# UVA-Computer-Vision-Lab/LabelAny3D

Measured on AMD Instinct MI355X. Metric: fitted 3D boxes/sec @640x480, higher is better.
Workload: dtype f64

## Files before the change

### labelany3d_amd/csrc/la3d_instance.hip

```cpp
#include <algorithm>
#include <atomic>
#include <chrono>
#include <cstdint>
#include <cstddef>
#include <cstring>
#include <mutex>
#include <type_traits>
#include <utility>
#include <vector>

#include "la3d_device.hpp"
#include "la3d_poly.hpp"
#include "la3d_engines.hpp"
#include "la3d_walks.hpp"
#include "la3d_stages.hpp"
#include "la3d_instance_phases.hpp"
#include "la3d_hull.hpp"

#ifndef LA3D_INSTANCE_DT
#define LA3D_INSTANCE_DT 0
#endif
#if LA3D_INSTANCE_DT == 0
using DepthT = float;
using KParams = la3d::FitParams;
#define LA3D_INSTANCE_FIT instance_fit
#elif LA3D_INSTANCE_DT == 1
using DepthT = la3d::d_f16;
using KParams = la3d::FitParams16;
#define LA3D_INSTANCE_FIT instance_fit_f16
#define fit_instances_kernel fit_instances_f16_kernel
#else
using DepthT = la3d::d_u16;
using KParams = la3d::FitParams16;
#define LA3D_INSTANCE_FIT instance_fit_u16
#define fit_instances_kernel fit_instances_u16_kernel
#endif

namespace {
__device__ inline const float* depth_planes(const FitParams& p, const FitParams&) { return p.depth; }
__device__ inline DepthCvt<float> depth_cvt(const FitParams&) { return {}; }
#if LA3D_INSTANCE_DT != 0
__device__ inline const DepthT* depth_planes(const FitParams&, const FitParams16& call) { return reinterpret_cast<const DepthT*>(call.depth16); }
__device__ inline DepthCvt<DepthT> depth_cvt(const FitParams16& call) {
  DepthCvt<DepthT> cv;
#if LA3D_INSTANCE_DT == 2
  cv.scale = call.d16_scale; cv.hole = call.d16_hole;
#endif
  return cv;
}
__device__ inline long long frame_depth_offset(const FitParams& call, int img) {
  const long long off_v = call.frames[img].depth_offset;
  return uniform_i64(off_v);
}
#endif
__device__ inline void sweep_sep_hull(const FitParams& p, const DepthT* __restrict__ dpl, const unsigned* bits, const unsigned short* list,
                                      int nactive, const double* Mg, unsigned* col, int wave, int lane, double px0, double pz0,
                                      double* acc, double* yext, int* cnt, const DepthCvt<DepthT> cv) {
  const int c = lane & 31, h4 = (lane >> 5) * 4;
  const double a00 = Mg[0], a02 = Mg[2], a11 = Mg[4], a12 = Mg[5];
  double s0 = acc[0], s1 = acc[1], s2 = acc[2], s3 = acc[3], s4 = acc[4], ylo = yext[0], yhi = yext[1];
  int n = *cnt;
  for (int e = wave; e < nactive; e += NWAVE) {
    const unsigned t = __builtin_amdgcn_readfirstlane((unsigned)list[e]);
    const int u = (int)(t & 0xffu) * 32 + c, v0 = (int)(t >> 8) * 8 + h4;
    const uint4 w = *reinterpret_cast<const uint4*>(bits + e * 8 + h4);
    const unsigned nib = ((w.x >> c) & 1u) | (((w.y >> c) & 1u) << 1) | (((w.z >> c) & 1u) << 2) | (((w.w >> c) & 1u) << 3);
    const double r0 = fma(a00, (double)u, a02);
    unsigned kmin = 0xffffffffu, kmax = 0u;
#pragma unroll
    for (int k = 0; k < 4; ++k) {
      const int v = v0 + k;
      if (((nib >> k) & 1u) && v < p.H) {
        const float df = depth_at<DepthT>(dpl, (long long)v * p.W + u, cv);
        if (finite_f32(df)) {
          const unsigned key = hull_key(__float_as_uint(df));
          kmin = min(kmin, key); kmax = max(kmax, key);
          const double d = (double)df;
          const double x = d * r0 - px0, z = d - pz0, y = d * fma(a11, (double)v, a12);
          s0 += x; s1 += z; s2 = fma(x, x, s2); s3 = fma(x, z, s3); s4 = fma(z, z, s4);
          ylo = fmin(ylo, y); yhi = fmax(yhi, y);
          n += 1;
        }
      }
    }
    if (kmin <= kmax) { atomicMin(col + u, kmin); atomicMax(col + p.W + u, kmax); }
  }
  acc[0] = s0; acc[1] = s1; acc[2] = s2; acc[3] = s3; acc[4] = s4; yext[0] = ylo; yext[1] = yhi;
  *cnt = n;
}

__device__ inline void hull_full_mask(Shared* sh, const FitParams& p, int inst, const DepthT* __restrict__ dpl, unsigned* bits, const unsigned short* list,
                                      int nactive, bool sep, const double* Mg, int nmask, int wave, int lane, const DepthCvt<DepthT> cv) {
  if (!sep) {
    if (tid_here(wave, lane) == 0) write_no_box(p, inst, LA3D_BOX_UNSUPPORTED, 0.0, NAN);
    return;
  }
  unsigned* col = bits + nactive * 8;
  double hacc[5] = {0, 0, 0, 0, 0}, yx[2] = {INFINITY, -INFINITY};
  int hcnt = 0;
  sweep_sep_hull(p, dpl, bits, list, nactive, Mg, col, wave, lane, 0.0, 0.0, hacc, yx, &hcnt, cv);
  stage_moments_to_axis(sh, p, inst, hacc, hcnt, nmask, tid_here(wave, lane), wave, lane, true);
  if (sh->redo) {
    __syncthreads();
    double piv[2];
    get_pivot(sh, piv);
#pragma unroll
    for (int i = 0; i < 5; ++i) hacc[i] = 0;
    hcnt = 0;
    sweep_sep_hull(p, dpl, bits, list, nactive, Mg, col, wave, lane, piv[0], piv[1], hacc, yx, &hcnt, cv);
    stage_moments_to_axis(sh, p, inst, hacc, hcnt, nmask, tid_here(wave, lane), wave, lane, false);
  }
  if (sh->st != LA3D_BOX_OK) return;
  const double ylo_w = wave_min(yx[0]), yhi_w = wave_max(yx[1]);
  if (lane == 0) { sh->part[wave][5] = ylo_w; sh->part[wave][6] = yhi_w; }
  __syncthreads();
  double* hh = hull_slot(p.geo, inst, hull_stride_bytes(false, p.W));
  unsigned* hcol = reinterpret_cast<unsigned*>(hh + HH_D);
  for (int i = tid_here(wave, lane); i < 2 * p.W; i += NT) hcol[i] = col[i];
  if (tid_here(wave, lane) == 0) {
    double ylo = INFINITY, yhi = -INFINITY;
    for (int w = 0; w < NWAVE; ++w) { ylo = fmin(ylo, sh->part[w][5]); yhi = fmax(yhi, sh->part[w][6]); }
    hull_handoff_header(hh, sh, ylo, yhi, Mg[0], Mg[2], 0.0);
  }
}

template <bool VEC, bool LDSMASK, bool SAMPLE, bool TILED, int SRC, bool HULL = false, bool FRAMES = false>
__global__ __launch_bounds__(NT, NT / 64) void fit_instances_kernel(const KParams p_call) {
  static_assert(!FRAMES || (VEC && LDSMASK && TILED && !HULL && (SRC == 1 || SRC == 2 || SRC == 3)), "frames calls: run lengths / polygons / bit planes, tiled form");
  FitParams p_frame;
  if constexpr (FRAMES) p_frame = p_call;
  const FitParams& p_block = p_call;
  const FitParams& p = FRAMES ? p_frame : p_block;
  extern __shared__ __attribute__((aligned(16))) unsigned char smem[];
  unsigned* bits = reinterpret_cast<unsigned*>(smem);
  Shared* sh = reinterpret_cast<Shared*>(smem + p_call.mask_lds_bytes);
  unsigned* prefix = reinterpret_cast<unsigned*>(smem + p_call.mask_lds_bytes + sizeof(Shared));
  unsigned short* list = reinterpret_cast<unsigned short*>(smem + p_call.mask_lds_bytes + sizeof(Shared));

  constexpr bool REBUILD_TID = TILED && !SAMPLE;
  const int tid_in = threadIdx.x;
  const int lane = REBUILD_TID ? (int)__builtin_amdgcn_mbcnt_hi(~0u, __builtin_amdgcn_mbcnt_lo(~0u, 0u)) : (tid_in & 63);
  const int wave = __builtin_amdgcn_readfirstlane(tid_in >> 6);
  const int tid = REBUILD_TID ? ((wave << 6) | lane) : tid_in;
#ifdef LA3D_TIMELINE
  const unsigned long long t_entry = wall_clock64();
#endif
  if (!FRAMES && !SAMPLE && p.order_self && (int)blockIdx.x < p.order_resident && !(p.order_self == 2 && blockIdx.x % 7 == 3)) {
    for (int ie = (int)blockIdx.x; ie < p.B; ie += p.order_resident) {
      if (ie != (int)blockIdx.x) __syncthreads();
      estimate_publish_wg<SRC == 3>(p, ie, sh, tid, wave, lane);
    }
  }
  const int inst = p.order_nch > 0 ? order_select<SRC == 3>(p, (int)blockIdx.x, sh, wave, lane) : xcd_remap(blockIdx.x, p.B);
  if (tid == 0) { sh->order_inst = inst; sh->sep_bad = 0; }
  if constexpr (HULL) { if (tid == 0) hull_slot(p.geo, inst, hull_stride_bytes(SAMPLE, p.W))[HH_STATE] = -1.0; }
  const int img = p.image_index ? p.image_index[inst] : inst;
  if constexpr (FRAMES) {
    if (!frame_geometry<true, SAMPLE>(p_frame, p_call, img) || (SRC == 3 && !frame_bits_offset_ok(p_call, inst))) {
      if (tid == 0) write_no_box(p, inst, LA3D_BOX_UNSUPPORTED, 0.0, NAN);
      return;
    }
  }
  const int HW = p.HW;
  const DepthT* dpl = depth_planes(p, p_call) + (long long)img * p.depth_plane_stride;
#if LA3D_INSTANCE_DT != 0
  if constexpr (FRAMES) dpl += frame_depth_offset(p_call, img);
#endif
  const DepthCvt<DepthT> cv = depth_cvt(p_call);
  const unsigned char* mpl = p.mask ? p.mask + (long long)inst * HW : nullptr;

  if (tid == NT - 1) {
    double Kinv[9], Rg[9];
    inv3_camera(p.K + (long long)img * p.k_stride, Kinv);
    sh->bad_ground = ground_rotation(p.ground ? p.ground + (long long)inst * 4 : nullptr, Rg);
#pragma unroll
    for (int i = 0; i < 3; ++i)
#pragma unroll
      for (int j = 0; j < 3; ++j) sh->M[i * 3 + j] = Rg[i] * Kinv[j] + Rg[3 + i] * Kinv[3 + j] + Rg[6 + i] * Kinv[6 + j];
#pragma unroll
    for (int i = 0; i < 9; ++i) sh->Rg[i] = Rg[i];
  }

#ifdef LA3D_TIMELINE
  double* tl = p.geo + 1024 + (long long)inst * 16;
#define LA3D_STAMP(k) do { if (tid == 0) tl[k] = (double)wall_clock64(); } while (0)
  if (tid == 0) { tl[7] = (double)blockIdx.x; tl[8] = (double)t_entry; sh->tl = tl; }
#else
#define LA3D_STAMP(k) do { } while (0)
#endif
  LA3D_STAMP(0);
  if (!SAMPLE && p.stagger_ticks > 0 && p.order_nch > 0 && blockIdx.x < 1024) {
    const unsigned long long t0 = wall_clock64();
    const unsigned g = blockIdx.x >> 8;
    const unsigned long long w = (unsigned long long)p.stagger_ticks * (g == 1 ? 13u : (g == 2 ? 29u : (g == 3 ? 47u : 0u))) / 16u;
    while (wall_clock64() - t0 < w) __builtin_amdgcn_s_sleep(32);
  }
  int my_draw = 0;
  if (SAMPLE && tid < LA3D_NSAMPLE) my_draw = p.sample_idx[(long long)inst * LA3D_NSAMPLE + tid];
  int nmask = 0;
  if constexpr (LDSMASK) nmask = mask_to_bits<VEC, SRC, FRAMES>(p, p_call, inst, mpl, bits, sh, list, TILED ? p.list_cap / 2 : 0, tid, wave, lane);
  __syncthreads();
  LA3D_STAMP(1);
  const int inst_p = __builtin_amdgcn_readfirstlane(sh->order_inst);
  if constexpr (FRAMES) frame_geometry<false, SAMPLE>(p_frame, p_call, p.image_index[inst_p]);
  const int tid_plain = tid;
#define tid (REBUILD_TID ? tid_here(wave, lane) : tid_plain)
  if (SRC != 0 && LDSMASK && p.filter_boundary >= 0) {
    if (!filter_keep<SRC>(p, sh, bits, inst_p, tid)) return;
  }
  double Mg[9];
#pragma unroll
  for (int i = 0; i < 9; ++i) Mg[i] = uniform_f64(sh->M[i]);
  LA3D_STAMP(13);

  bool sampled = false;
  int ntot = 0;
  if (SAMPLE) {
    const int wsum = wave_sum_i(nmask);
    if (lane == 0) sh->nmask[wave] = wsum;
    __syncthreads();
    for (int w = 0; w < NWAVE; ++w) ntot += sh->nmask[w];
    sampled = HULL || ntot > LA3D_NSAMPLE;
  }

  constexpr bool LK = TILED && !SAMPLE;
  const bool sep_cam = LK && (HULL || !p.sep_off) && Mg[1] == 0.0 && Mg[3] == 0.0 && Mg[6] == 0.0 && Mg[7] == 0.0 && Mg[8] == 1.0;
  TileList tiles;
  if (TILED && !sampled) {
    if constexpr (FRAMES) frame_rcp_ntx(p_frame);
    tiles = build_tile_list<LK>(p, sh, bits, list, sep_cam, tid, wave, lane);
    LA3D_STAMP(15);
    __syncthreads();
  }
  const int nactive = tiles.nactive, nfull = tiles.nfull, compact = tiles.compact;
  const bool sep = tiles.sep;

  if constexpr (HULL && LK) {
    hull_full_mask(sh, p, inst_p, dpl, bits, list, nactive, sep, Mg, nmask, wave, lane, cv);
    return;
  }

  if constexpr (LK) {
    if (sep) {
      LA3D_STAMP(2);
      unsigned* col = bits + nactive * 8;
      double sacc[5] = {0, 0, 0, 0, 0}, yx[2] = {INFINITY, -INFINITY};
      unsigned unsafe = 0u;
      if (p.H & 7) sweep_sep<true>(p, dpl, bits, list, nactive, Mg, col, wave, lane, sacc, yx, &unsafe, 0, nfull, cv);
      else sweep_sep<false>(p, dpl, bits, list, nactive, Mg, col, wave, lane, sacc, yx, &unsafe, 0, nfull, cv);
      if (__ballot(unsafe >= 0x7f800000u) != 0ull && lane == 0) sh->sep_bad = 1;
      const double ylo_w = uniform_f64(wave_min(yx[0])), yhi_w = uniform_f64(wave_max(yx[1]));
      LA3D_STAMP(3);
      stage_moments_to_axis(sh, p, inst_p, sacc, nmask, nmask, tid, wave, lane, true);
      LA3D_STAMP(4);
      if (!(sh->redo || sh->sep_bad)) {
        if (sh->st != LA3D_BOX_OK) return;
        double N0[3], N2[3], ext[6];
        yaw_rows(sh, Mg, N0, N2);
        sep_col_extents(col, p.W, N0, N2, tid, ext);
        ext[2] = ylo_w; ext[3] = yhi_w;
        LA3D_STAMP(5);
        if constexpr (FRAMES) frame_proj(p_frame, p_call, inst_p);
        stage_extents_to_box(sh, p, inst_p, ext, tid, wave, lane);
        stage_status_aux(sh, p, inst_p, tid);
        LA3D_STAMP(6);
        return;
      }
      __syncthreads();
    }
  }

  bool cull = false;
  int rng_words = 0;
  if constexpr (LK) {
    if (compact) {
      rng_words = cull_rng_words(nactive);
      cull = nactive >= p.cull_min && nactive <= CULL_MAXT;
      if (!cull) {
        unsigned short* surv = reinterpret_cast<unsigned short*>(bits + nactive * 8);
#pragma clang loop vectorize(disable) interleave(disable) unroll(disable)
        for (int t = tid; t < nactive; t += NT) surv[t] = (unsigned short)t;
      }
    }
  }

  LA3D_STAMP(2);
  double acc[5] = {0, 0, 0, 0, 0};
  int cnt = 0;
  double px = 0, py = 0, pz = 0;
  bool pok = false;

  if (SAMPLE) {
    if (sampled) {
      sample_pick<HULL, FRAMES, DepthT>(p, sh, bits, prefix, dpl, cv, Mg, ntot, my_draw, tid, wave, lane, acc, &cnt, &px, &py, &pz, &pok);
    }
  }
  bool checked = !TILED;
  if (!sampled) {
    if (TILED) {
      constexpr bool SP = !SAMPLE;
      const bool specA = SP && Mg[6] == 0.0 && Mg[7] == 0.0 && Mg[8] == 1.0;
      if (LK && cull) {
        if (specA) sweep_tiled<0, false, true, SP>(p, dpl, bits, list, nactive, Mg, Mg + 3, Mg + 6, wave, lane, acc, &cnt, nullptr, compact, rng_words, -1, nfull, cv);
        else sweep_tiled<0, false, true>(p, dpl, bits, list, nactive, Mg, Mg + 3, Mg + 6, wave, lane, acc, &cnt, nullptr, compact, rng_words, -1, nfull, cv);
      } else {
        if (specA) sweep_tiled<0, false, false, SP>(p, dpl, bits, list, nactive, Mg, Mg + 3, Mg + 6, wave, lane, acc, &cnt, nullptr, compact, rng_words, -1, nfull, cv);
        else sweep_tiled<0, false>(p, dpl, bits, list, nactive, Mg, Mg + 3, Mg + 6, wave, lane, acc, &cnt, nullptr, compact, rng_words, -1, nfull, cv);
      }
      cnt = nmask;
    }
    else sweep<VEC, LDSMASK, 0>(p, dpl, mpl, bits, Mg, Mg + 3, Mg + 6, wave, lane, acc, &cnt, &nmask, nullptr, cv);
  }

  LA3D_STAMP(3);
  stage_moments_to_axis(sh, p, inst_p, acc, cnt, nmask, tid, wave, lane, true);
  if (sh->redo) {
    __syncthreads();
#pragma unroll
    for (int i = 0; i < 5; ++i) acc[i] = 0;
    cnt = 0;
    if (sampled) {
      if (pok) {
        const double x = px - pivot_ptr(sh)[0], z = pz - pivot_ptr(sh)[1];
        acc[0] = x; acc[1] = z; acc[2] = x * x; acc[3] = x * z; acc[4] = z * z;
        cnt = 1;
      }
    } else if (TILED) {
      if (sh->redo == 2) {
        pivot_pass(p, dpl, bits, list, nactive, Mg, Mg + 6, wave, lane, compact, pivot_ptr(sh), acc, &cnt, cv);
      } else {
        checked = true;
        if (LK && cull) sweep_tiled<0, true, true>(p, dpl, bits, list, nactive, Mg, Mg + 3, Mg + 6, wave, lane, acc, &cnt, nullptr, compact, rng_words, -1, nfull, cv);
        else sweep_tiled<0, true>(p, dpl, bits, list, nactive, Mg, Mg + 3, Mg + 6, wave, lane, acc, &cnt, nullptr, compact, rng_words, -1, nfull, cv);
      }
    } else {
      double piv[2];
      get_pivot(sh, piv);
      sweep<VEC, LDSMASK, 0, true>(p, dpl, mpl, bits, Mg, Mg + 3, Mg + 6, wave, lane, acc, &cnt, &nmask, piv, cv);
    }
    stage_moments_to_axis(sh, p, inst_p, acc, cnt, nmask, tid, wave, lane, false);
  }
  LA3D_STAMP(4);
  if (sh->st != LA3D_BOX_OK) return;

  if constexpr (HULL && SAMPLE) {
    double* hh = hull_slot(p.geo, inst_p, hull_stride_bytes(true, p.W));
    if (tid_plain < HULL_SMALL) {
      double* q = hh + HH_D + 3 * tid_plain;
      q[0] = pok ? px : NAN; q[1] = pok ? py : NAN; q[2] = pok ? pz : NAN;
    }
    if (tid_plain == 0) hull_handoff_header(hh, sh, 0.0, 0.0, 0.0, 0.0, (double)min(ntot, LA3D_NSAMPLE));
    return;
  }

  double ext[6] = {INFINITY, -INFINITY, INFINITY, -INFINITY, INFINITY, -INFINITY};
  if (sampled) {
    if (pok) {
      const double x2 = sh->cyaw * px + sh->syaw * pz;
      const double z2 = -sh->syaw * px + sh->cyaw * pz;
      ext[0] = ext[1] = x2;
      ext[2] = ext[3] = py;
      ext[4] = ext[5] = z2;
    }
  } else {
    double N0[3], N2[3];
    yaw_rows(sh, Mg, N0, N2);
    int d0 = 0, d1 = 0;
    if (TILED) {
      unsigned* qh = &sh->qhead;
      int nsurv = -1;
      if constexpr (LK) {
        if (compact) nsurv = nactive;
        if (cull) {
          nsurv = checked ? cull_plan<true>(sh, p, dpl, bits, list, nactive, rng_words, N0, Mg + 3, N2, tid, wave, lane, ext, cv)
                          : cull_plan<false>(sh, p, dpl, bits, list, nactive, rng_words, N0, Mg + 3, N2, tid, wave, lane, ext, cv);
        }
      }
      if (checked) sweep_tiled<1, true>(p, dpl, bits, list, nactive, N0, Mg + 3, N2, wave, lane, ext, &d0, qh, compact, rng_words, nsurv, 0, cv);
      else if (!SAMPLE && Mg[3] == 0.0) sweep_tiled<1, false, false, !SAMPLE>(p, dpl, bits, list, nactive, N0, Mg + 3, N2, wave, lane, ext, &d0, qh, compact, rng_words, nsurv, 0, cv);
      else sweep_tiled<1, false>(p, dpl, bits, list, nactive, N0, Mg + 3, N2, wave, lane, ext, &d0, qh, compact, rng_words, nsurv, 0, cv);
    }
    else sweep<VEC, LDSMASK, 1>(p, dpl, mpl, bits, N0, Mg + 3, N2, wave, lane, ext, &d0, &d1, nullptr, cv);
  }
  LA3D_STAMP(5);
  if constexpr (FRAMES) frame_proj(p_frame, p_call, inst_p);
  stage_extents_to_box(sh, p, inst_p, ext, tid, wave, lane);
  stage_status_aux(sh, p, inst_p, tid);
  LA3D_STAMP(6);
}
#undef tid

template <bool VEC, bool SAMPLE, int SRC>
int launch_hull_inst(const KParams& p, size_t lds, hipStream_t s) {
  auto kern = fit_instances_kernel<VEC, true, SAMPLE, !SAMPLE, SRC, true>;
  allow_big_lds(reinterpret_cast<const void*>(kern));
  hipLaunchKernelGGL(kern, dim3(p.B), dim3(NT), lds, s, p);
  const int rc = check_launch("fit_instances_kernel (hull)");
  if (rc != LA3D_SUCCESS) return rc;
  return la3d::hull_finish_launch(p, SAMPLE, s);
}
template <int SRC> using src_t = std::integral_constant<int, SRC>;
template <bool DECODED, bool NO_U8 = false, typename F>
int with_src(const KParams& p, F&& f) {
  if constexpr (DECODED) {
    if (p.mask_bits != nullptr) return f(src_t<3>());
    if (p.rle_counts != nullptr) return f(src_t<1>());
    if (NO_U8 || p.poly_xy != nullptr) return f(src_t<2>());
  }
  if constexpr (NO_U8) return LA3D_ERR_UNSUPPORTED;
  else return f(src_t<0>());
}
template <bool VEC, bool SAMPLE>
int launch_hull(const KParams& p, size_t lds, hipStream_t s) {
  return with_src<true>(p, [&](auto src) { return launch_hull_inst<VEC || decltype(src)::value != 0, SAMPLE, decltype(src)::value>(p, lds, s); });
}

template <bool VEC, bool LDSMASK, bool SAMPLE, bool TILED, int SRC, bool FRAMES = false>
int launch_fit_inst(const KParams& p_in, size_t lds, hipStream_t s, void* workspace) {
  auto kern = fit_instances_kernel<VEC, LDSMASK, SAMPLE, TILED, SRC, false, FRAMES>;
  allow_big_lds(reinterpret_cast<const void*>(kern));
  KParams p = p_in;
  if (workspace && VEC && !SAMPLE && p.B > 256 && p.B <= ORDER_MAX_B && balance_enabled(p) && (!FRAMES || p.area_hint)) {
    int wg_per_cu = 2048 / NT;
    const int by_lds = (int)((160 * 1024) / (lds ? lds : 1));
    if (by_lds < wg_per_cu) wg_per_cu = by_lds;
    if (wg_per_cu >= 1 && p.B <= BALANCE_MAX_ROUNDS * wg_per_cu * 256) {
      p.order_nch = (p.B + ORDER_CHUNK - 1) / ORDER_CHUNK;
      p.order_resident = wg_per_cu * 256;
      const OrderKeyScale k = order_key_scale(p);
      if (p.area_hint) {
        p.order_shift = k.shift;
      } else {
        unsigned* est = static_cast<unsigned*>(workspace);
        p.order_keys = est;
        bool self = config().order_self != 0 && wg_per_cu * 256 >= 256;
#ifdef LA3D_TIMELINE
        self = false;
#endif
        if (self && stream_capturing(s)) self = false;
        if (self) {
          p.order_self = config().order_self; p.est_step = k.step; p.order_shift = k.shift;
          p.order_flags = reinterpret_cast<unsigned long long*>(static_cast<unsigned char*>(workspace) + (((size_t)p.B * 4 + 255) & ~(size_t)255));
          const unsigned long long t = (unsigned long long)std::chrono::steady_clock::now().time_since_epoch().count();
          p.order_nonce = (t * 0x9E3779B97F4A7C15ull) ^ (unsigned long long)reinterpret_cast<uintptr_t>(workspace) ^ 0xA5A5A5A55A5A5A5Aull;
        } else if (SRC == 3) {
          hipLaunchKernelGGL(size_estimate_bits_kernel, dim3((p.B + 3) / 4), dim3(256), 0, s, static_cast<const FitParams&>(p), k.shift, est);
        } else {
          hipLaunchKernelGGL(size_estimate_kernel, dim3((p.B + 3) / 4), dim3(256), 0, s, p.mask, p.rle_counts, p.rle_offsets, p.poly_xy,
                             p.poly_ring_off, p.poly_inst_rings, p.B, p.HW, k.step, k.shift, est, nullptr);
        }
      }
    }
  }
  hipLaunchKernelGGL(kern, dim3(p.B), dim3(NT), lds, s, p);
  return check_launch("fit_instances_kernel");
}


template <bool VEC, bool LDSMASK, bool SAMPLE, bool TILED = false>
int launch_fit(const KParams& p, size_t lds, hipStream_t s, void* workspace = nullptr) {
  return with_src<LDSMASK>(p, [&](auto src) { return launch_fit_inst<VEC, LDSMASK, SAMPLE, TILED, decltype(src)::value>(p, lds, s, workspace); });
}

template <bool SAMPLE>
int launch_fit_frames(const KParams& p, size_t lds, hipStream_t s, void* workspace) {
  return with_src<true, true>(p, [&](auto src) { return launch_fit_inst<true, true, SAMPLE, true, decltype(src)::value, true>(p, lds, s, workspace); });
}

}

namespace la3d {
int LA3D_INSTANCE_FIT(KParams p, const CallFacts& f, hipStream_t s, void* workspace, const char* who) {
  const int H = p.H, W = p.W, B = p.B;
  const bool vec = f.vec, ldsmask = f.ldsmask;
  if (f.sample && !ldsmask) return refuse(who, "reference-subsample mode needs the bit image in LDS (H*W <= 1048576)", LA3D_ERR_UNSUPPORTED);
  const size_t blocks = f.sample ? (size_t)rank_prefix_bytes(p.nwords) : 0;
  auto lds_with = [&](size_t list_bytes) { return f.lds + std::max({list_bytes, blocks, f.poly_stage}); };
  p.ntx = W / 32; p.nty = (H + 7) / 8;
  p.rcp_ntx = 1.0f / (float)(p.ntx > 0 ? p.ntx : 1);
  p.tiles_per_wave = (p.ntx * p.nty + NWAVE - 1) / NWAVE;
  const bool tiled_frame = ldsmask && vec && W % 32 == 0 && p.ntx <= 255 && p.nty <= 255;
  if (f.sample) {
    if (lds_with(0) > 160 * 1024 - 256) return refuse(who, "reference-subsample mode: frame too large for LDS", LA3D_ERR_UNSUPPORTED);
    if (f.method == LA3D_METHOD_CONVEX_HULL) {
      p.geo = static_cast<double*>(f.hull_area);
      return vec ? launch_hull<true, true>(p, lds_with(0), s) : launch_hull<false, true>(p, lds_with(0), s);
    }
    if (tiled_frame) {
      int budget = 0;
      const long cap = tiled_list_cap<true>(p.mask_lds_bytes, p.nwords, p.ntx * p.nty, &budget);
      if (cap >= 64 && budget <= 160 * 1024 - 256) {
        p.list_cap = (int)cap;
        if (f.frames) return launch_fit_frames<true>(p, lds_with((size_t)cap * 2), s, nullptr);
        return launch_fit<true, true, true, true>(p, lds_with((size_t)cap * 2), s);
      }
    }
    if (f.frames)
      return refuse(who, "reference-subsample mode: bounds outside the tiled form: H <= 2040, W <= 8160, and bit image + rank "
                         "prefix + 64 tile-list entries within one workgroup's LDS (160 KiB)", LA3D_ERR_UNSUPPORTED);
    return vec ? launch_fit<true, true, true>(p, lds_with(0), s) : launch_fit<false, true, true>(p, lds_with(0), s);
  }
  if (tiled_frame) {
    const long cap = tiled_list_cap<false>(p.mask_lds_bytes, p.nwords, p.ntx * p.nty);
    if (cap >= 64) {
      p.list_cap = (int)cap;
      const size_t lds = lds_with((size_t)cap * 2);
      if (f.method == LA3D_METHOD_CONVEX_HULL) {
        p.geo = static_cast<double*>(f.hull_area);
        return launch_hull<true, false>(p, lds, s);
      }
      if (f.frames) return launch_fit_frames<false>(p, lds, s, workspace);
      if (p.mask != nullptr && B > 256) {
        double us = 256.0 * (double)p.HW / 6.4e6;
        if (config().stagger_us >= 0) us = config().stagger_us;
        p.stagger_ticks = (int)(us * 100.0);
      }
      return launch_fit<true, true, false, true>(p, lds, s, workspace);
    }
  }
  if (f.frames)
    return refuse(who, "bounds outside the tiled form: H <= 2040, W <= 8160, and bit image + 64 tile-list entries within one "
                       "workgroup's LDS (160 KiB)", LA3D_ERR_UNSUPPORTED);
  if (f.method == LA3D_METHOD_CONVEX_HULL) {
    return hull_refuse_launch(p, s);
  }
  if (ldsmask) return vec ? launch_fit<true, true, false>(p, lds_with(0), s, workspace) : launch_fit<false, true, false>(p, lds_with(0), s);
  return vec ? launch_fit<true, false, false>(p, lds_with(0), s) : launch_fit<false, false, false>(p, lds_with(0), s);
}
}
```

### labelany3d_amd/csrc/la3d_instance_phases.hpp

```cpp
#pragma once
#include "la3d_device.hpp"
#include "la3d_poly.hpp"
#include "la3d_hull.hpp"

using namespace la3d;

namespace {
template <bool VEC, int SRC, bool FRAMES>
__device__ inline int mask_to_bits(const FitParams& p, const FitParams& call, int inst, const unsigned char* mpl, unsigned* bits, Shared* sh,
                                   void* stage, int stage_words, int tid, int wave, int lane) {
  const int HW = p.HW;
  int nmask = 0;
  if constexpr (SRC == 1) {
    const long long o0 = p.rle_offsets[inst];
    nmask = rle_to_bits<NT>(p.rle_counts + o0, (int)(p.rle_offsets[inst + 1] - o0), bits, p.nwords, p.H, p.W, sh->scan, tid,
                            static_cast<unsigned*>(stage), stage_words, p.frame_w);
  } else if constexpr (SRC == 2) {
    nmask = poly_to_bits<NT>(p.poly_xy, p.poly_ring_off, p.poly_inst_rings[inst], p.poly_inst_rings[inst + 1],
                             static_cast<PolySide*>(stage), sh->scan, bits, p.nwords, p.H, p.W, tid, p.frame_w);
  } else if constexpr (SRC == 3) {
    if constexpr (FRAMES) nmask = bits_plane_to_lds<NT>(p.mask_bits + frame_bits_offset(call, inst), bits, p.nwords, HW, 1, tid);
    else nmask = bits_plane_to_lds<NT>(p.mask_bits + (long long)inst * p.bits_plane_stride, bits, p.nwords, HW, p.bits_vec, tid);
  } else {
    unsigned short* b16 = reinterpret_cast<unsigned short*>(bits);
    const int ngroups = (HW + 15) >> 4;
    if (VEC) {
      const u32x4* m4 = reinterpret_cast<const u32x4*>(mpl);
      constexpr int P0U = 4;
      unsigned seen = 0;
#pragma unroll P0U
      for (int g = tid; g < ngroups; g += NT) {
        const u32x4 w = __builtin_nontemporal_load(m4 + g);
        const unsigned lo = __builtin_amdgcn_udot4(w.y, 0x80402010u, __builtin_amdgcn_udot4(w.x, 0x08040201u, 0u, false), false);
        const unsigned hi = __builtin_amdgcn_udot4(w.w, 0x80402010u, __builtin_amdgcn_udot4(w.z, 0x08040201u, 0u, false), false);
        const unsigned pat = lo | (hi << 8);
        seen |= (w.x | w.y) | (w.z | w.w);
        b16[g] = (unsigned short)pat;
        nmask += __popc(pat);
      }
      const unsigned long long odd = __ballot((seen & 0xfefefefeu) != 0);
      if (lane == 0) sh->scan[wave] = odd != 0 ? 1u : 0u;
      __syncthreads();
      unsigned general = 0;
#pragma unroll
      for (int w = 0; w < NWAVE; ++w) general |= sh->scan[w];
      if (general) {
        nmask = 0;
#pragma unroll 4
        for (int g = tid; g < ngroups; g += NT) {
          const u32x4 w = m4[g];
          const unsigned pat = nz16(w.x, w.y, w.z, w.w);
          b16[g] = (unsigned short)pat;
          nmask += __popc(pat);
        }
      }
    } else {
      for (int g = tid; g < ngroups; g += NT) {
        unsigned pat = 0;
        for (int k = 0; k < 16; ++k) {
          const int i = g * 16 + k;
          if (i < HW && mpl[i]) pat |= 1u << k;
        }
        b16[g] = (unsigned short)pat;
        nmask += __popc(pat);
      }
    }
    if ((ngroups & 1) && tid == 0) b16[ngroups] = 0;
  }
  return nmask;
}

template <int SRC>
__device__ inline bool filter_keep(const FitParams& p, Shared* sh, const unsigned* bits, int inst, int tid) {
  int st4[4];
  bits_filter_stats<NT>(bits, p.H, p.frame_w, p.filter_boundary, reinterpret_cast<int*>(sh->part), tid, st4, p.W);
  if (p.filter_stats && tid < 4) (p.filter_stats + (long long)inst * 4)[tid] = st4[tid];
  const int height = SRC == 1 ? st4[1] : (SRC == 3 && !p.bits_span) ? st4[1] : st4[2];
  const bool keep = 16 * height > p.H && st4[3] < p.filter_max_edge && st4[0] >= p.filter_min_area;
  if (!keep && tid == 0) write_no_box(p, inst, LA3D_BOX_FILTERED, 0.0, (double)st4[0]);
  return keep;
}

struct TileList {
  int nactive = 0, nfull = 0, compact = 0;
  bool sep = false;
};

template <bool WHOLE_ROWS, bool LK>
__device__ inline void classify_tiles(const FitParams& p, const unsigned* bits, int tbeg, int tend, int lane, unsigned long long* bal,
                                      unsigned (*wrd)[8], int* wcount, int* fcount, unsigned* fl) {
#pragma unroll
  for (int k = 0; k < 4; ++k) {
    const int t = tbeg + k * 64 + lane;
    unsigned any = 0, all = 0xffffffffu;
    if (t < tend) {
      const int ty = (int)(((float)t + 0.5f) * p.rcp_ntx), tx = t - ty * p.ntx;
      const int rmax = p.H - 1 - ty * 8;
      const unsigned* bw = bits + (ty * 8) * p.ntx + tx;
#pragma unroll
      for (int rr = 0; rr < 8; ++rr) {
        const unsigned w = bw[(WHOLE_ROWS ? rr : min(rr, rmax)) * p.ntx];
        any |= w;
        if constexpr (LK) { wrd[k][rr] = (WHOLE_ROWS || rr <= rmax) ? w : 0u; all &= wrd[k][rr]; }
      }
    }
    bal[k] = __ballot(any != 0);
    *wcount += __popcll(bal[k]);
    if constexpr (LK) {
      const bool f = t < tend && all == 0xffffffffu;
      *fcount += __popcll(__ballot(f));
      *fl |= (f ? 1u : 0u) << k;
    }
  }
}

template <bool LK>
__device__ inline TileList build_tile_list(const FitParams& p, Shared* sh, unsigned* bits, unsigned short* list, bool sep_cam, int tid, int wave, int lane) {
  TileList tl;
  const int ntiles = p.ntx * p.nty, per = p.tiles_per_wave;
  const int tbeg = wave * per, tend = min(tbeg + per, ntiles);
  int base = 0;
  if (per <= 256) {
    unsigned long long bal[4];
    unsigned wrd[LK ? 4 : 1][8];
    int wcount = 0, fcount = 0;
    unsigned fl = 0;
    if ((p.H & 7) == 0) classify_tiles<true, LK>(p, bits, tbeg, tend, lane, bal, wrd, &wcount, &fcount, &fl);
    else classify_tiles<false, LK>(p, bits, tbeg, tend, lane, bal, wrd, &wcount, &fcount, &fl);
    if (lane == 0) sh->scan[wave] = (unsigned)wcount | ((unsigned)fcount << 16);
    __syncthreads();
    LA3D_SUBSTAMP(sh, 14);
    int fbase = 0;
    for (int w = 0; w < NWAVE; ++w) {
      const int c = (int)(sh->scan[w] & 0xffffu), f = (int)(sh->scan[w] >> 16);
      if (w < wave) { base += c - f; fbase += f; }
      tl.nactive += c;
      tl.nfull += f;
    }
    if (tl.nactive > p.list_cap) {
      tl.nactive = -1;
      tl.nfull = 0;
    } else {
      if constexpr (LK) tl.compact = (tl.nactive * 32 + cull_rng_words(tl.nactive) * 4 <= p.mask_lds_bytes) ? 1 : 0;
      int foff = fbase, poff = tl.nfull + base;
#pragma unroll
      for (int k = 0; k < 4; ++k) {
        const bool isf = LK && ((fl >> k) & 1u);
        const unsigned long long bf = LK ? __ballot(isf) : 0ull, bp = bal[k] & ~bf, lt = (1ull << lane) - 1ull;
        if ((bal[k] >> lane) & 1ull) {
          const int t = tbeg + k * 64 + lane;
          const int ty = (int)(((float)t + 0.5f) * p.rcp_ntx), tx = t - ty * p.ntx;
          const int idx = isf ? foff + __popcll(bf & lt) : poff + __popcll(bp & lt);
          list[idx] = (unsigned short)((ty << 8) | tx);
          if constexpr (LK) if (tl.compact) {
            uint4* e = reinterpret_cast<uint4*>(bits) + 2 * idx;
            e[0] = make_uint4(wrd[k][0], wrd[k][1], wrd[k][2], wrd[k][3]);
            e[1] = make_uint4(wrd[k][4], wrd[k][5], wrd[k][6], wrd[k][7]);
          }
        }
        foff += __popcll(bf); poff += __popcll(bp);
      }
      if constexpr (LK) if (tl.compact) {
        if (sep_cam && tl.nactive * 32 + sep_col_words(p.W) * 4 <= p.mask_lds_bytes) {
          tl.sep = true;
          unsigned* col = bits + tl.nactive * 8;
#pragma clang loop vectorize(disable) interleave(disable) unroll(disable)
          for (int u = tid; u < p.W; u += NT) { col[u] = 0xffffffffu; col[p.W + u] = 0u; }
        }
      }
    }
  } else {
#pragma unroll 1
    for (int pass = 0; pass < 2; ++pass) {
      int wcount = 0;
      for (int t0 = tbeg; t0 < tend; t0 += 64) {
        const int t = t0 + lane;
        unsigned any = 0, packed = 0;
        if (t < tend) {
          const int ty = t / p.ntx, tx = t - ty * p.ntx;
          const int rows = min(8, p.H - ty * 8);
          const unsigned* bw = bits + (ty * 8) * p.ntx + tx;
          for (int rr = 0; rr < rows; ++rr) any |= bw[rr * p.ntx];
          packed = ((unsigned)ty << 8) | (unsigned)tx;
        }
        const unsigned long long bal = __ballot(any != 0);
        if (pass == 1 && any) list[base + wcount + __popcll(bal & ((1ull << lane) - 1ull))] = (unsigned short)packed;
        wcount += __popcll(bal);
      }
      if (pass == 0) {
        if (lane == 0) sh->scan[wave] = (unsigned)wcount;
        __syncthreads();
        for (int w = 0; w < NWAVE; ++w) {
          const int c = (int)sh->scan[w];
          if (w < wave) base += c;
          tl.nactive += c;
        }
        if (tl.nactive > p.list_cap) { tl.nactive = -1; break; }
      }
    }
  }
  return tl;
}

template <bool HULL, bool FRAMES, typename DepthT>
__device__ inline void sample_pick(const FitParams& p, Shared* sh, const unsigned* bits, unsigned* prefix, const DepthT* __restrict__ dpl,
                                          const DepthCvt<DepthT> cv, const double* Mg, int ntot, int my_draw, int tid, int wave, int lane,
                                          double* acc, int* cnt, double* ppx, double* ppy, double* ppz, bool* ppok) {
  const int nblk = (p.nwords + 31) >> 5;
  unsigned run0 = 0;
  for (int b0 = 0; b0 < nblk; b0 += NT) {
    const int blk = b0 + tid;
    unsigned local = 0;
    if (blk < nblk) {
      const int w0 = blk << 5, wn = min(32, p.nwords - w0);
      if (wn == 32) {
        const uint4* q = reinterpret_cast<const uint4*>(bits + w0);
#pragma unroll
        for (int i = 0; i < 8; ++i) { const uint4 v = q[i]; local += __popc(v.x) + __popc(v.y) + __popc(v.z) + __popc(v.w); }
      } else {
        for (int i = 0; i < wn; ++i) local += __popc(bits[w0 + i]);
      }
    }
    unsigned incl = local;
#pragma unroll
    for (int o = 1; o < 64; o <<= 1) {
      const unsigned t = __shfl_up(incl, o);
      if (lane >= o) incl += t;
    }
    if (lane == 63) sh->scan[wave] = incl;
    __syncthreads();
    unsigned base = run0, tot = 0;
    for (int w = 0; w < NWAVE; ++w) { const unsigned c = sh->scan[w]; if (w < wave) base += c; tot += c; }
    if (blk < nblk) prefix[blk] = base + incl - local;
    run0 += tot;
    __syncthreads();
  }
  if (tid < (HULL ? min(ntot, LA3D_NSAMPLE) : LA3D_NSAMPLE)) {
    int r = (HULL && ntot <= LA3D_NSAMPLE) ? tid : my_draw;
    r = r < 0 ? 0 : (r >= ntot ? ntot - 1 : r);
    int lo = 0, hi = nblk - 1;
    while (lo < hi) {
      const int mid = (lo + hi + 1) >> 1;
      if (prefix[mid] <= (unsigned)r) lo = mid; else hi = mid - 1;
    }
    int k = r - (int)prefix[lo];
    lo <<= 5;
    unsigned w = 0;
    if (lo + 32 <= p.nwords) {
      uint4 q[8];
#pragma unroll
      for (int i = 0; i < 8; ++i) q[i] = reinterpret_cast<const uint4*>(bits + lo)[i];
      int sel = 0;
      bool found = false;
#pragma unroll
      for (int i = 0; i < 32; ++i) {
        const unsigned wi = (i & 3) == 0 ? q[i >> 2].x : (i & 3) == 1 ? q[i >> 2].y : (i & 3) == 2 ? q[i >> 2].z : q[i >> 2].w;
        const int c = __popc(wi);
        const bool here = !found && k < c;
        if (here) { w = wi; sel = i; }
        found = found || here;
        if (!found) k -= c;
      }
      lo += sel;
    } else {
      const int wend = p.nwords - 1;
      for (; lo < wend; ++lo) {
        const int c = __popc(bits[lo]);
        if (k < c) break;
        k -= c;
      }
      w = bits[lo];
    }
    for (; k > 0; --k) w &= w - 1;
    const unsigned i = (unsigned)lo * 32u + (unsigned)(__ffs((int)w) - 1);
    const float df = depth_at<DepthT>(dpl, i, cv);
    unsigned u, v;
    pix_uv(i, p.W, FRAMES ? 1.0f / (float)p.W : p.rcpW, &u, &v);
    const double ud = (double)u, vd = (double)v;
    const bool pok = finite_f32(df);
    const double d = pok ? (double)df : 0.0;
    const double px = d * fma(Mg[0], ud, fma(Mg[1], vd, Mg[2]));
    const double py = d * fma(Mg[3], ud, fma(Mg[4], vd, Mg[5]));
    const double pz = d * fma(Mg[6], ud, fma(Mg[7], vd, Mg[8]));
    *ppx = px; *ppy = py; *ppz = pz; *ppok = pok;
    if (pok) {
      acc[0] = px; acc[1] = pz; acc[2] = px * px; acc[3] = px * pz; acc[4] = pz * pz;
      *cnt = 1;
    }
  }
}

__device__ inline void hull_handoff_header(double* hh, const Shared* sh, double ylo, double yhi, double a00, double a02, double npts) {
  hh[HH_NVALID] = (double)sh->n_valid; hh[HH_NM] = (double)sh->nm; hh[HH_CYAW] = sh->cyaw; hh[HH_SYAW] = sh->syaw;
  hh[HH_GAP] = sh->gap; hh[HH_YLO] = ylo; hh[HH_YHI] = yhi;
  for (int i = 0; i < 9; ++i) hh[HH_RG + i] = sh->Rg[i];
  hh[HH_A00] = a00; hh[HH_A02] = a02; hh[HH_NPTS] = npts;
  hh[HH_STATE] = 0.0;
}
}
```

Baseline: 11.64 million.

## Stream u8 masks directly into tile-major LDS bits with depth prefetch touch

For u8 tiled masks, adds a streaming converter that packs 16 mask bytes into a 16-bit pattern with dot4 instructions, using nontemporal loads, and writes the result straight into a tile-major LDS layout. A fallback pass reruns the general nonzero conversion if any byte is not 0/1. Tile classification then reads each tile as two contiguous uint4 loads, and the row-major layout is restored when compact mode is off. For sparse waves it also issues early depth loads to warm the cache. The intent is to cut the conversion and strided tile-gather cost, at the price of an extra barrier and more complex layout handling.

```diff
diff --git a/labelany3d_amd/csrc/la3d_instance.hip b/labelany3d_amd/csrc/la3d_instance.hip
--- a/labelany3d_amd/csrc/la3d_instance.hip
+++ b/labelany3d_amd/csrc/la3d_instance.hip
@@ -197,9 +197,12 @@
   }
   int my_draw = 0;
   if (SAMPLE && tid < LA3D_NSAMPLE) my_draw = p.sample_idx[(long long)inst * LA3D_NSAMPLE + tid];
+  constexpr bool TM = SRC == 0 && VEC && LDSMASK && TILED && !SAMPLE;
   int nmask = 0;
-  if constexpr (LDSMASK) nmask = mask_to_bits<VEC, SRC, FRAMES>(p, p_call, inst, mpl, bits, sh, list, TILED ? p.list_cap / 2 : 0, tid, wave, lane);
+  if constexpr (TM) nmask = u8_stream_to_bits(p, mpl, bits, sh, tid, wave, lane);
+  else if constexpr (LDSMASK) nmask = mask_to_bits<VEC, SRC, FRAMES>(p, p_call, inst, mpl, bits, sh, list, TILED ? p.list_cap / 2 : 0, tid, wave, lane);
   __syncthreads();
+  if constexpr (TM) nmask = u8_general_rerun(p, mpl, bits, sh, nmask, tid);
   LA3D_STAMP(1);
   const int inst_p = __builtin_amdgcn_readfirstlane(sh->order_inst);
   if constexpr (FRAMES) frame_geometry<false, SAMPLE>(p_frame, p_call, p.image_index[inst_p]);
@@ -228,7 +231,7 @@
   TileList tiles;
   if (TILED && !sampled) {
     if constexpr (FRAMES) frame_rcp_ntx(p_frame);
-    tiles = build_tile_list<LK>(p, sh, bits, list, sep_cam, tid, wave, lane);
+    tiles = build_tile_list<LK, TM, DepthT>(p, sh, bits, list, sep_cam, tid, wave, lane, dpl);
     LA3D_STAMP(15);
     __syncthreads();
   }
diff --git a/labelany3d_amd/csrc/la3d_instance_phases.hpp b/labelany3d_amd/csrc/la3d_instance_phases.hpp
--- a/labelany3d_amd/csrc/la3d_instance_phases.hpp
+++ b/labelany3d_amd/csrc/la3d_instance_phases.hpp
@@ -6,6 +6,14 @@
 using namespace la3d;
 
 namespace {
+__device__ inline bool tile_major_image(const FitParams& p) { return (p.H & 7) == 0 && p.tiles_per_wave <= 256; }
+__device__ inline int tile_major_half(int v, int q, int ntx) { return ((((v >> 3) * ntx + (q >> 1)) << 4) | ((v & 7) << 1)) | (q & 1); }
+__device__ inline unsigned pat16_01(const u32x4& w) {
+  const unsigned lo = __builtin_amdgcn_udot4(w.y, 0x80402010u, __builtin_amdgcn_udot4(w.x, 0x08040201u, 0u, false), false);
+  const unsigned hi = __builtin_amdgcn_udot4(w.w, 0x80402010u, __builtin_amdgcn_udot4(w.z, 0x08040201u, 0u, false), false);
+  return lo | (hi << 8);
+}
+
 template <bool VEC, int SRC, bool FRAMES>
 __device__ inline int mask_to_bits(const FitParams& p, const FitParams& call, int inst, const unsigned char* mpl, unsigned* bits, Shared* sh,
                                    void* stage, int stage_words, int tid, int wave, int lane) {
@@ -70,6 +78,63 @@
   return nmask;
 }
 
+__device__ inline int u8_stream_to_bits(const FitParams& p, const unsigned char* mpl, unsigned* bits, Shared* sh, int tid, int wave, int lane) {
+  unsigned short* b16 = reinterpret_cast<unsigned short*>(bits);
+  const u32x4* m4 = reinterpret_cast<const u32x4*>(mpl);
+  const int ngroups = (p.HW + 15) >> 4;
+  constexpr int P0U = 4;
+  unsigned seen = 0;
+  int nmask = 0;
+  if (tile_major_image(p)) {
+    const int gpr = p.W >> 4, dv = NT / gpr, dq = NT - dv * gpr;
+    int v = tid / gpr, q = tid - v * gpr;
+#pragma unroll P0U
+    for (int g = tid; g < ngroups; g += NT) {
+      const u32x4 w = __builtin_nontemporal_load(m4 + g);
+      const unsigned pat = pat16_01(w);
+      seen |= (w.x | w.y) | (w.z | w.w);
+      b16[tile_major_half(v, q, p.ntx)] = (unsigned short)pat;
+      nmask += __popc(pat);
+      v += dv; q += dq;
+      if (q >= gpr) { q -= gpr; ++v; }
+    }
+  } else {
+#pragma unroll P0U
+    for (int g = tid; g < ngroups; g += NT) {
+      const u32x4 w = __builtin_nontemporal_load(m4 + g);
+      const unsigned pat = pat16_01(w);
+      seen |= (w.x | w.y) | (w.z | w.w);
+      b16[g] = (unsigned short)pat;
+      nmask += __popc(pat);
+    }
+  }
+  const unsigned long long odd = __ballot((seen & 0xfefefefeu) != 0);
+  if (lane == 0) sh->nmask[wave] = odd != 0 ? 1 : 0;
+  return nmask;
+}
+
+__device__ inline int u8_general_rerun(const FitParams& p, const unsigned char* mpl, unsigned* bits, const Shared* sh, int nmask, int tid) {
+  int general = 0;
+#pragma unroll
+  for (int w = 0; w < NWAVE; ++w) general |= sh->nmask[w];
+  if (!general) return nmask;
+  unsigned short* b16 = reinterpret_cast<unsigned short*>(bits);
+  const u32x4* m4 = reinterpret_cast<const u32x4*>(mpl);
+  const int ngroups = (p.HW + 15) >> 4, gpr = p.W >> 4;
+  const bool tm = tile_major_image(p);
+  nmask = 0;
+#pragma unroll 4
+  for (int g = tid; g < ngroups; g += NT) {
+    const u32x4 w = m4[g];
+    const unsigned pat = nz16(w.x, w.y, w.z, w.w);
+    const int v = g / gpr;
+    b16[tm ? tile_major_half(v, g - v * gpr, p.ntx) : g] = (unsigned short)pat;
+    nmask += __popc(pat);
+  }
+  __syncthreads();
+  return nmask;
+}
+
 template <int SRC>
 __device__ inline bool filter_keep(const FitParams& p, Shared* sh, const unsigned* bits, int inst, int tid) {
   int st4[4];
@@ -114,8 +179,50 @@
   }
 }
 
-template <bool LK>
-__device__ inline TileList build_tile_list(const FitParams& p, Shared* sh, unsigned* bits, unsigned short* list, bool sep_cam, int tid, int wave, int lane) {
+__device__ inline void classify_tiles_tm(const unsigned* bits, int tbeg, int tend, int lane, unsigned long long* bal, unsigned (*wrd)[8],
+                                         int* wcount, int* fcount, unsigned* fl) {
+#pragma unroll
+  for (int k = 0; k < 4; ++k) {
+    const int t = tbeg + k * 64 + lane;
+    unsigned any = 0, all = 0u;
+    if (t < tend) {
+      const uint4 a = reinterpret_cast<const uint4*>(bits)[2 * t], b = reinterpret_cast<const uint4*>(bits)[2 * t + 1];
+      wrd[k][0] = a.x; wrd[k][1] = a.y; wrd[k][2] = a.z; wrd[k][3] = a.w;
+      wrd[k][4] = b.x; wrd[k][5] = b.y; wrd[k][6] = b.z; wrd[k][7] = b.w;
+      any = ((a.x | a.y) | (a.z | a.w)) | ((b.x | b.y) | (b.z | b.w));
+      all = ((a.x & a.y) & (a.z & a.w)) & ((b.x & b.y) & (b.z & b.w));
+    }
+    bal[k] = __ballot(any != 0);
+    *wcount += __popcll(bal[k]);
+    const bool f = all == 0xffffffffu;
+    *fcount += __popcll(__ballot(f));
+    *fl |= (f ? 1u : 0u) << k;
+  }
+}
+
+constexpr int TOUCH_TILES = 8;
+template <typename DT>
+__device__ inline unsigned depth_touch(const FitParams& p, const DT* __restrict__ dpl, const unsigned long long* bal, int tbeg, int lane) {
+  int mine = -1, n = 0;
+#pragma unroll
+  for (int k = 0; k < 4; ++k) {
+    for (unsigned long long m = bal[k]; m != 0ull; m &= m - 1ull) {
+      if ((lane >> 3) == n) mine = tbeg + k * 64 + (__ffsll((long long)m) - 1);
+      ++n;
+    }
+  }
+  unsigned word = 0u;
+  if (mine >= 0) {
+    const int ty = (int)(((float)mine + 0.5f) * p.rcp_ntx), tx = mine - ty * p.ntx;
+    const int row = min(ty * 8 + (lane & 7), p.H - 1);
+    word = *reinterpret_cast<const unsigned*>(dpl + ((long long)row * p.W + tx * 32));
+  }
+  return word;
+}
+
+template <bool LK, bool TM = false, typename DT = float>
+__device__ inline TileList build_tile_list(const FitParams& p, Shared* sh, unsigned* bits, unsigned short* list, bool sep_cam, int tid, int wave, int lane,
+                                           const DT* __restrict__ dpl = nullptr) {
   TileList tl;
   const int ntiles = p.ntx * p.nty, per = p.tiles_per_wave;
   const int tbeg = wave * per, tend = min(tbeg + per, ntiles);
@@ -125,8 +232,17 @@
     unsigned wrd[LK ? 4 : 1][8];
     int wcount = 0, fcount = 0;
     unsigned fl = 0;
-    if ((p.H & 7) == 0) classify_tiles<true, LK>(p, bits, tbeg, tend, lane, bal, wrd, &wcount, &fcount, &fl);
-    else classify_tiles<false, LK>(p, bits, tbeg, tend, lane, bal, wrd, &wcount, &fcount, &fl);
+    if constexpr (TM) {
+      if ((p.H & 7) == 0) classify_tiles_tm(bits, tbeg, tend, lane, bal, wrd, &wcount, &fcount, &fl);
+      else classify_tiles<false, LK>(p, bits, tbeg, tend, lane, bal, wrd, &wcount, &fcount, &fl);
+    } else {
+      if ((p.H & 7) == 0) classify_tiles<true, LK>(p, bits, tbeg, tend, lane, bal, wrd, &wcount, &fcount, &fl);
+      else classify_tiles<false, LK>(p, bits, tbeg, tend, lane, bal, wrd, &wcount, &fcount, &fl);
+    }
+    unsigned touched = 0u;
+    if constexpr (TM && TOUCH_TILES > 0) {
+      if (wcount > 0 && wcount <= TOUCH_TILES) touched = depth_touch<DT>(p, dpl, bal, tbeg, lane);
+    }
     if (lane == 0) sh->scan[wave] = (unsigned)wcount | ((unsigned)fcount << 16);
     __syncthreads();
     LA3D_SUBSTAMP(sh, 14);
@@ -168,6 +284,21 @@
           for (int u = tid; u < p.W; u += NT) { col[u] = 0xffffffffu; col[p.W + u] = 0u; }
         }
       }
+    }
+    if constexpr (TM) {
+      if ((p.H & 7) == 0 && !tl.compact) {
+#pragma unroll
+        for (int k = 0; k < 4; ++k) {
+          const int t = tbeg + k * 64 + lane;
+          if (t < tend) {
+            const int ty = (int)(((float)t + 0.5f) * p.rcp_ntx), tx = t - ty * p.ntx;
+            unsigned* bw = bits + (ty * 8) * p.ntx + tx;
+#pragma unroll
+            for (int rr = 0; rr < 8; ++rr) bw[rr * p.ntx] = wrd[k][rr];
+          }
+        }
+      }
+      if constexpr (TOUCH_TILES > 0) asm volatile("" : : "v"(touched));
     }
   } else {
 #pragma unroll 1
```

Result: no change. 11.62 million (-0.2%).
